# ppwwyyxx/OpenPano

Measured on AMD Instinct MI355X. Metric: SIFT keypoints+desc/sec and all-pairs matches/sec at 1/2/4/8 GPUs, higher is better.
Workload: dtype f32; 1 GPU; BASELINE config 4 restated: 38 unordered 1300x867 views per GPU (x1 GPUs = a 38-image job); seeded synthetic views (ope~; images_per_gpu=38, images_in_job=38

## Files before the change

include/openpano_hip.h:

```cpp
#ifndef OPENPANO_HIP_H
#define OPENPANO_HIP_H
#include <stddef.h>
#include <stdint.h>
#ifdef __cplusplus
extern "C" {
#endif

typedef enum {
	OP_OK = 0,
	OP_ERR_INVALID = -1,
	OP_ERR_HIP = -2,
	OP_ERR_CAPACITY = -3,
	OP_ERR_UNSUPPORTED = -4,
	OP_ERR_NO_FEATURE = -5
} op_status;

const char* op_last_error(void);
int op_abi_version(void);

typedef struct op_config {
	int SIFT_WORKING_SIZE, NUM_OCTAVE, NUM_SCALE;
	float SCALE_FACTOR, GAUSS_SIGMA;
	int GAUSS_WINDOW_FACTOR;
	float JUDGE_EXTREMA_DIFF_THRES, CONTRAST_THRES, PRE_COLOR_THRES, EDGE_RATIO;
// ... 53 lines not shown
typedef struct op_sift_dump op_sift_dump;
int op_sift_staged(op_ctx* ctx, const op_config* cfg, const op_image* img, op_sift_dump** out);
void op_sift_dump_free(op_sift_dump* d);
int op_sift_dump_working_dims(const op_sift_dump* d, int* h, int* w);
int op_sift_dump_octave_dims(const op_sift_dump* d, int oct, int* h, int* w);
int op_sift_dump_plane(op_ctx* ctx, const op_sift_dump* d, int kind, int oct, int s, float* out);
int op_sift_dump_raw_count(const op_sift_dump* d, int oct, int s);
int op_sift_dump_raw(const op_sift_dump* d, int oct, int s, int* xy);
int op_sift_dump_kp_count(const op_sift_dump* d, int which);
int op_sift_dump_kp(const op_sift_dump* d, int which, int* ints, double* real, float* fl);
int op_sift_dump_desc(const op_sift_dump* d, float* desc, double* coor);

int op_debug_math(op_ctx* ctx, int which, const float* x, const float* y, int n, float* out);
int op_debug_set_raw_capacity(op_ctx* ctx, int cap);
int op_debug_set_desc_list_cap(op_ctx* ctx, int floats);

typedef struct op_matches op_matches;
int op_match_pairs(op_ctx* ctx, const op_config* cfg, const op_features* f,
		const int* pairs, int npairs, op_matches** out);
int op_matches_count(const op_matches* m, int p);
int op_matches_copy(const op_matches* m, int p, int* idx_pairs);
int op_matches_copy_all(const op_matches* m, int* idx_pairs, int64_t* offsets);
const int* op_matches_device_list(const op_matches* m);
int64_t op_matches_total(const op_matches* m);
int op_matches_from_host(const int* const* idx_pairs, const int* counts, int npairs, op_matches** out);
int op_matches_concat(op_ctx* ctx, const op_matches* a, const op_matches* b, op_matches** out);
void op_matches_free(op_matches* m);

typedef struct op_group op_group;
int op_group_create(const int* devices, int ndev, op_group** out);
// ... 88 lines not shown
```

openpano_amd/csrc/capi.hip:

```cpp
#include "internal.hpp"
#include <cstring>

static thread_local std::string g_last_error;
void op_set_error(const std::string& msg) { g_last_error = msg; }

static hipEvent_t take_event(op_ctx* c) {
	if (!c->ev_pool.empty()) { hipEvent_t e = c->ev_pool.back(); c->ev_pool.pop_back(); return e; }
	hipEvent_t e = nullptr;
	if (hipEventCreate(&e) != hipSuccess) return nullptr;
	return e;
}
ProfScope::ProfScope(op_ctx* ctx, const char* label): c(ctx) {
	if (!c->profiling || (!c->prof_only.empty() && c->prof_only != label)) return;
	stage = c->prof_stage(label);
	a = take_event(c); b = take_event(c);
	if (a) hipEventRecord(a, c->stream);
}
ProfScope::~ProfScope() {
	if (stage < 0 || !a || !b) return;
	hipEventRecord(b, c->stream);
	c->pending.push_back({stage, a, b});
}
#include <chrono>
static double now_ms() { return std::chrono::duration<double, std::milli>(std::chrono::steady_clock::now().time_since_epoch()).count(); }
// ... 185 lines not shown
	if (n == 0) return OP_OK;
	HIPCHK(hipSetDevice(c->device));
	float *dx = nullptr, *dy = nullptr, *dout = nullptr;
	HIPCHK(hipMalloc(&dx, sizeof(float) * n));
	HIPCHK(hipMalloc(&dy, sizeof(float) * n));
	HIPCHK(hipMalloc(&dout, sizeof(float) * n));
	HIPCHK(hipMemcpyAsync(dx, x, sizeof(float) * n, hipMemcpyHostToDevice, c->stream));
	HIPCHK(hipMemcpyAsync(dy, y ? y : x, sizeof(float) * n, hipMemcpyHostToDevice, c->stream));
	HIPCHK(launch_debug_math(which, dx, dy, n, dout, c->stream));
	HIPCHK(hipMemcpyAsync(out, dout, sizeof(float) * n, hipMemcpyDeviceToHost, c->stream));
	HIPCHK(hipStreamSynchronize(c->stream));
	hipFree(dx); hipFree(dy); hipFree(dout);
	return OP_OK;
}

}
```

openpano_amd/csrc/internal.hpp:

```cpp
#pragma once
#include <hip/hip_runtime.h>
#include <stdint.h>
#include <string>
#include <vector>
#include "openpano_hip.h"

#define OP_MAX_OCT 8
#define OP_MAX_SCALE 12
#define OP_MAX_KCENTER 15

void op_set_error(const std::string& msg);
struct op_ctx;
void op_ctx_release_workspace(op_ctx* c);
#define OP_FAIL(code, msg) do { op_set_error(msg); return (code); } while (0)
#define HIPCHK(expr) do { hipError_t e_ = (expr); if (e_ != hipSuccess) { \
	op_set_error(std::string(#expr) + ": " + hipGetErrorString(e_)); return OP_ERR_HIP; } } while (0)

struct ProfStage { std::string label; double total_ms = 0; long calls = 0; };
struct op_ctx {
	int device = 0;
	int num_cu = 256;
	hipStream_t stream = nullptr;
	bool owns_stream = false;
	bool profiling = false;
// ... 64 lines not shown
#include <functional>
void host_parallel_for(int n, const std::function<void(int)>& body, int grain = 1);

hipError_t pool_alloc(void** p, size_t bytes);
void pool_free(void* p);
void pool_trim();

struct OctDesc {
	int h, w;
	int tiles_x, tiles_y, tile_begin;
	int rw_nb, rw_nseg;
	long long off;
	long long plane;
};

struct SiftPlan {
	int n;
	int sh, sw;
	int wh, ww;
	int noct, nscale;
	OctDesc oct[OP_MAX_OCT];
	int total_tiles;
	long long ws_stride;
	float* ws;
	float* work;
	const void* const* srcs;
	int src_u8;
	int* zero;
	int zero_n;
	int num_cu;
	float kern[OP_MAX_SCALE][2 * OP_MAX_KCENTER + 1];
	int kcenter[OP_MAX_SCALE];
	int halo;
	int rows_ok;
	int rw_seg;
	int rw_items;
	float kpair[3][7][2];
	float pre_color_thres, judge_thres, contrast_thres, edge_ratio, offset_thres;
	int calc_offset_depth;
	float gauss_sigma, scale_factor, ori_radius;
	int ori_smooth, desc_scale_factor, desc_int_factor;
	int desc_list_cap;
};

__host__ __device__ inline long long plane_off_grey(const OctDesc& o) { return o.off; }
// ... 6 lines not shown
	float dir, sf;
	int src;
	int pad;
};

#define OP_DESC_LIST_CAP 640
#define OP_RW_OWN 240
#define OP_RW_SEG_DEFAULT 24
#define OP_RW_SEG_MIN 16
#define OP_RW_SEG_MAX 40
#define OP_PYR_TW 64
#ifndef OP_PYR_TH
#define OP_PYR_TH 16
#endif

hipError_t launch_grey_octaves(const SiftPlan& p, bool write_work, hipStream_t st);
hipError_t launch_pyramid(const SiftPlan& p, int* raw , int* raw_count , int cap, hipStream_t st);
hipError_t launch_magort_plane(const SiftPlan& p, int img, int oct, int s, float* mag, float* ort, hipStream_t st);
hipError_t launch_refine(const SiftPlan& p, const int* raw, const int* raw_count, int cap, int expect,
		KeyPoint* refined , int* refined_count, hipStream_t st);
#define OP_OCNT_STRIDE 32
hipError_t launch_orientation(const SiftPlan& p, const KeyPoint* refined, const int* refined_count, int cap, int expect,
		float* dirs , int* ndirs , int* per_image ,
		KeyPoint* sorted , int* slot_of , hipStream_t st);
hipError_t launch_expand_oriented(const SiftPlan& p, const KeyPoint* sorted, const int* slot_of, const int* refined_count, int cap,
		const float* dirs, const int* ndirs, const int* per_image , long long* total, int* count_out ,
		KeyPoint* oriented, long long oriented_cap, hipStream_t st);
hipError_t launch_descriptor(const SiftPlan& p, const KeyPoint* oriented, const long long* total ,
		long long cap, float* desc, double* coor, double* real, hipStream_t st);
hipError_t launch_debug_math(int which, const float* x, const float* y, int n, float* out, hipStream_t st);
// ... 1 lines not shown
```

openpano_amd/csrc/pyramid.hip:

```cpp
#include "internal.hpp"
#include "devmath.hpp"

namespace {

__device__ __forceinline__ void resize_coord(int d, float inv_f, int srcn, int& s, float& r) {
	float rr = ((float)d + 0.5f) * inv_f - 0.5f;
	int ss = (int)floorf(rr);
	rr -= (float)ss;
	if (ss < 0) { ss = 0; rr = 0.f; }
	else if (ss + 1 >= srcn) { ss = srcn - 2; rr = 1.f; }
	s = ss; r = rr;
}

__device__ __forceinline__ float bilerp(float p00, float p01, float p10, float p11, float rx, float irx, float ry, float iry) {
	return rx * (p11 * ry + p10 * iry) + irx * (p01 * ry + p00 * iry);
}

#ifndef OP_GREY_WR
#define OP_GREY_WR 14
#endif
constexpr int WT = 64, WR = OP_GREY_WR;
constexpr int WP = WT + 1 + 2;

typedef float f32x4_a4 __attribute__((ext_vector_type(4), aligned(4)));
typedef float f32x2_a4 __attribute__((ext_vector_type(2), aligned(4)));
#define OP_GLOBAL __attribute__((address_space(1)))
__device__ __forceinline__ void src_run6(const float* s, long long i, const float*, float (&t)[6]) {
	const OP_GLOBAL float* g = (const OP_GLOBAL float*)s + i;
	const f32x4_a4 a = *(const OP_GLOBAL f32x4_a4*)g; const f32x2_a4 b = *(const OP_GLOBAL f32x2_a4*)(g + 4);
	t[0] = a.x; t[1] = a.y; t[2] = a.z; t[3] = a.w; t[4] = b.x; t[5] = b.y;
}
__device__ __forceinline__ void src_run6(const unsigned char* s, long long i, const float* lut, float (&t)[6]) {
#pragma unroll
	for (int k = 0; k < 6; ++k) t[k] = lut[((const OP_GLOBAL unsigned char*)s)[i + k]];
}

__device__ __forceinline__ float third(float s) { return (float)((double)s * (1.0 / 3.0)); }

constexpr int TR = 24, TC = 72;

#ifdef OP_GREY_WAVES
#define OP_GREY_ATTR __attribute__((amdgpu_waves_per_eu(OP_GREY_WAVES, OP_GREY_WAVES)))
#else
#define OP_GREY_ATTR
#endif
template <typename SrcT>
__global__ void __launch_bounds__(256) OP_GREY_ATTR k_grey_octaves(SiftPlan p, int write_work) {
	__shared__ float s_rgb[3][(WR + 1) * WP];
	__shared__ float s_lut[256];
	__shared__ int s_ri[TR], s_ci[TC];
	__shared__ float s_rw[TR], s_cw[TC];
	__shared__ long long s_ro[TR];
	const unsigned ntx = (unsigned)(p.ww + WT - 1) / WT, nty = (unsigned)(p.wh + WR - 1) / WR;
	const unsigned ntile = ntx * nty * (unsigned)p.n, per = (ntile + 7u) >> 3;
	const unsigned lin = (blockIdx.x & 7u) * per + (blockIdx.x >> 3);
	if (lin >= ntile) return;
	const int img = (int)(lin / (ntx * nty));
	const unsigned trem = lin - (unsigned)img * (ntx * nty);
	const int tx0 = (int)(trem % ntx) * WT, ty0 = (int)(trem / ntx) * WR;
	const int tid = threadIdx.x;
	const SrcT* src = (const SrcT*)p.srcs[img];
	if (blockIdx.x == 0 && p.zero)
		for (int i = tid; i < p.zero_n; i += 256) p.zero[i] = 0;
	if (sizeof(SrcT) == 1) s_lut[tid] = (float)((double)(float)tid / 255.0);
	{
		const float fx = (float)p.wh / (float)p.sh, fy = (float)p.ww / (float)p.sw;
		const float ifx = 1.f / fx, ify = 1.f / fy;
		if (tid < WR + 1) {
			int sx = -1; float rx = 0.f;
			if (ty0 + tid < p.wh) resize_coord(ty0 + tid, ifx, p.sh, sx, rx);
			s_ri[tid] = sx; s_rw[tid] = rx; s_ro[tid] = (long long)sx * p.sw * 3;
		} else if (tid >= 64 && tid < 64 + WT + 1) {
			const int c = tid - 64;
			int sy = -1; float ry = 0.f;
			if (tx0 + c < p.ww) resize_coord(tx0 + c, ify, p.sw, sy, ry);
			s_ci[c] = sy < 0 ? -1 : sy * 3; s_cw[c] = ry;
		}
		__syncthreads();
		constexpr int NE = ((WR + 1) * (WT + 1) + 255) / 256;
		float t0[NE][6], t1[NE][6];
		bool live[NE];
#pragma unroll
		for (int k = 0; k < NE; ++k) {
			const int e = tid + 256 * k < (WR + 1) * (WT + 1) ? tid + 256 * k : 0;
			const int r = e / (WT + 1), c = e % (WT + 1);
			const int sx = s_ri[r], sy3 = s_ci[c];
			live[k] = sx >= 0 && sy3 >= 0;
			const long long i0 = live[k] ? s_ro[r] + sy3 : 0, i1 = i0 + (long long)p.sw * 3;
			src_run6(src, i0, s_lut, t0[k]); src_run6(src, i1, s_lut, t1[k]);
		}
#pragma unroll
		for (int k = 0; k < NE; ++k) {
			const int e = tid + 256 * k;
			if (e >= (WR + 1) * (WT + 1)) break;
			const int r = e / (WT + 1), c = e % (WT + 1);
			float v0 = 0.f, v1 = 0.f, v2 = 0.f;
			if (live[k]) {
				const float rx = s_rw[r], ry = s_cw[c];
				const float irx = 1.0f - rx, iry = 1.0f - ry;
				v0 = bilerp(t0[k][0], t0[k][3], t1[k][0], t1[k][3], rx, irx, ry, iry);
				v1 = bilerp(t0[k][1], t0[k][4], t1[k][1], t1[k][4], rx, irx, ry, iry);
				v2 = bilerp(t0[k][2], t0[k][5], t1[k][2], t1[k][5], rx, irx, ry, iry);
				if (write_work && r < WR && c < WT) {
					float* dst = p.work + (((long long)img * p.wh + ty0 + r) * p.ww + tx0 + c) * 3;
					dst[0] = v0; dst[1] = v1; dst[2] = v2;
				}
			}
			s_rgb[0][r * WP + c] = v0; s_rgb[1][r * WP + c] = v1; s_rgb[2][r * WP + c] = v2;
		}
	}
	__syncthreads();
	float* ws = p.ws + (long long)img * p.ws_stride;
	{
		const int c = tid & (WT - 1), col = tx0 + c;
		float* g0 = ws + plane_off_grey(p.oct[0]) + (long long)ty0 * p.ww + col;
		if (col < p.ww)
			for (int r = tid >> 6; r < WR && ty0 + r < p.wh; r += 4)
				g0[(long long)r * p.ww] = third(s_rgb[0][r * WP + c] + s_rgb[1][r * WP + c] + s_rgb[2][r * WP + c]);
	}
	for (int o = 1; o < p.noct; ++o) {
		const OctDesc od = p.oct[o];
		const float fx = (float)od.h / (float)p.wh, fy = (float)od.w / (float)p.ww;
		const float ifx = 1.f / fx, ify = 1.f / fy;
		int r_lo = (int)floorf(((float)ty0 + 0.5f) * fx - 0.5f) - 1, r_hi = (int)ceilf(((float)(ty0 + WR) + 0.5f) * fx - 0.5f) + 2;
		int c_lo = (int)floorf(((float)tx0 + 0.5f) * fy - 0.5f) - 1, c_hi = (int)ceilf(((float)(tx0 + WT) + 0.5f) * fy - 0.5f) + 2;
		r_lo = r_lo < 0 ? 0 : r_lo; c_lo = c_lo < 0 ? 0 : c_lo;
		r_hi = r_hi > od.h ? od.h : r_hi; c_hi = c_hi > od.w ? od.w : c_hi;
		const int nr = r_hi - r_lo, nc = c_hi - c_lo;
		if (nr <= 0 || nc <= 0) continue;
		const bool tables = nr <= TR && nc <= TC;
		__syncthreads();
		if (tables) {
			if (tid < nr) {
				int sx; float rx;
				resize_coord(r_lo + tid, ifx, p.wh, sx, rx);
				const int lr = sx - ty0;
				s_ri[tid] = (lr >= 0 && lr < WR) ? lr : -1; s_rw[tid] = rx;
			} else if (tid >= 64 && tid - 64 < nc) {
				int sy; float ry;
				resize_coord(c_lo + tid - 64, ify, p.ww, sy, ry);
				const int lc = sy - tx0;
				s_ci[tid - 64] = (lc >= 0 && lc < WT) ? lc : -1; s_cw[tid - 64] = ry;
			}
		}
		__syncthreads();
		float* go = ws + plane_off_grey(od);
		const float inv_nc = 1.0f / (float)nc;
		for (int e = tid; e < nr * nc; e += 256) {
			int q = (int)(((float)e + 0.5f) * inv_nc), rem = e - q * nc;
			if (rem < 0) { --q; rem += nc; } else if (rem >= nc) { ++q; rem -= nc; }
			const int dr = r_lo + q, dc = c_lo + rem;
			int lr, lc; float rx, ry;
			if (tables) { lr = s_ri[q]; lc = s_ci[rem]; rx = s_rw[q]; ry = s_cw[rem]; }
			else {
				int sx, sy;
				resize_coord(dr, ifx, p.wh, sx, rx);
				resize_coord(dc, ify, p.ww, sy, ry);
				lr = sx - ty0; lc = sy - tx0;
				if (lr >= WR) lr = -1;
				if (lc >= WT) lc = -1;
			}
			if (lr < 0 || lc < 0) continue;
			const float irx = 1.0f - rx, iry = 1.0f - ry;
			const int b = lr * WP + lc;
			const float r = bilerp(s_rgb[0][b], s_rgb[0][b + 1], s_rgb[0][b + WP], s_rgb[0][b + WP + 1], rx, irx, ry, iry);
			const float g = bilerp(s_rgb[1][b], s_rgb[1][b + 1], s_rgb[1][b + WP], s_rgb[1][b + WP + 1], rx, irx, ry, iry);
			const float bl = bilerp(s_rgb[2][b], s_rgb[2][b + 1], s_rgb[2][b + WP], s_rgb[2][b + WP + 1], rx, irx, ry, iry);
			go[(long long)dr * od.w + dc] = third(r + g + bl);
		}
	}
}

constexpr int TW = OP_PYR_TW, TH = OP_PYR_TH;
constexpr int GR = TH + 2, GC = TW + 2;
constexpr int PG = TH == 16 ? 75 : GC + 1;
constexpr int PV = GR + (GR % 2 == 0 ? 1 : 2);
constexpr int NPX = TW * TH / 256;
constexpr int NHALO = 2 * GC + 2 * TH;
static_assert(TW == 64 && TH % 4 == 0 && NHALO <= 256, "tile shape");
constexpr int RV = TH == 32 ? 12 : (TH == 24 ? 9 : 6);
constexpr int RH = TH == 32 ? 10 : (TH == 24 ? 8 : 6);
static_assert(((GR + RV - 1) / RV) * (GC + 12) <= 256 && ((GC + RH - 1) / RH) * GR <= 256, "blocking must fit 256 threads at halo 6");

// ... 575 lines not shown
		case 2: r = opdev::sinf_glibc(x[i]); break;
		case 3: r = opdev::hypotf_glibc(x[i], y[i]); break;
		default: r = opdev::fast_atan_plus_pi(y[i], x[i]); break;
	}
	out[i] = r;
}

}

size_t pyramid_lds_bytes(int halo) {
	const int NR = GR + 2 * halo, NC = GC + 2 * halo;
	return sizeof(float) * ((size_t)NR * NC + (size_t)vt_rows(halo) * PV + 4 * (size_t)GR * PG);
}

hipError_t launch_grey_octaves(const SiftPlan& p, bool write_work, hipStream_t st) {
	const unsigned ntile = (unsigned)((p.ww + WT - 1) / WT) * (unsigned)((p.wh + WR - 1) / WR) * (unsigned)p.n;
	dim3 grid(((ntile + 7u) >> 3) << 3);
	if (p.src_u8) hipLaunchKernelGGL(k_grey_octaves<unsigned char>, grid, dim3(256), 0, st, p, write_work ? 1 : 0);
	else hipLaunchKernelGGL(k_grey_octaves<float>, grid, dim3(256), 0, st, p, write_work ? 1 : 0);
	return hipGetLastError();
}

hipError_t launch_magort_plane(const SiftPlan& p, int img, int oct, int s, float* mag, float* ort, hipStream_t st) {
	const long long n = p.oct[oct].plane;
	hipLaunchKernelGGL(k_magort_plane, dim3((unsigned)((n + 255) / 256)), dim3(256), 0, st, p, img, oct, s, mag, ort);
	return hipGetLastError();
}

hipError_t launch_pyramid(const SiftPlan& p, int* raw, int* raw_count, int cap, hipStream_t st) {
	size_t lds = pyramid_lds_bytes(p.halo);
	{
// ... 20 lines not shown
```

openpano_amd/csrc/sift_host.hip:

```cpp
#include "internal.hpp"
#include <algorithm>
#include <array>
#include <cmath>
#include <cstring>
#include <map>
#include <memory>
#include <mutex>
#include <thread>

size_t pyramid_lds_bytes(int halo);

namespace {

struct DevBuf {
	void* p = nullptr; size_t cap = 0;
	hipError_t ensure(size_t bytes) {
		if (bytes <= cap) return hipSuccess;
		if (p) { hipError_t e = hipFree(p); if (e != hipSuccess) return e; p = nullptr; cap = 0; }
		size_t want = bytes + bytes / 8;
		hipError_t e = hipMalloc(&p, want);
		if (e != hipSuccess) return e;
		cap = want;
		return hipSuccess;
	}
	void release() { if (p) hipFree(p); p = nullptr; cap = 0; }
};

}

struct Workspace {
	DevBuf ws, work, srcs, staging, raw, counts, refinedA, refinedB, slot_of, dirs, ndirs, oriented;
	void* pinned = nullptr; size_t pinned_cap = 0;
	std::vector<const void*> srcs_last; void* srcs_dev = nullptr;
	long long last_total = 0;
	int last_raw_max = 0, last_refined_max = 0;
	int raw_cap = 16384;
	int desc_list_cap = OP_DESC_LIST_CAP;
	void release() {
		ws.release(); work.release(); srcs.release(); staging.release(); raw.release(); counts.release();
		refinedA.release(); refinedB.release(); slot_of.release(); dirs.release(); ndirs.release(); oriented.release();
		if (pinned) hipHostFree(pinned); pinned = nullptr; pinned_cap = 0;
		srcs_last.clear(); srcs_dev = nullptr;
	}
};

static std::map<op_ctx*, Workspace*> g_ws;
static std::mutex g_ws_mu;

static Workspace* ctx_workspace(op_ctx* c) {
	std::lock_guard<std::mutex> lk(g_ws_mu);
	auto it = g_ws.find(c);
	if (it != g_ws.end()) return it->second;
	Workspace* w = new Workspace;
	g_ws[c] = w;
	return w;
// ... 67 lines not shown
		kernel[0] = 1;
		float exp_coeff = (float)(-1.0 / (sigma * sigma * 2)), wsum = 1;
		for (int i = 1; i <= center; i++)
			wsum += (kernel[i] = std::exp((float)(i * i) * exp_coeff)) * 2;
		float fac = (float)(1.0 / wsum);
		kernel[0] = fac;
		for (int i = 1; i <= center; i++)
			kernel[-i] = (kernel[i] *= fac);
		p.kcenter[s] = center;
		p.halo = std::max(p.halo, center);
		sigma *= cfg.SCALE_FACTOR;
	}
	return 0;
}

int build_plan(const op_config& cfg, int n, int sh, int sw, SiftPlan& p, int num_cu = 256) {
	memset(&p, 0, sizeof(p));
	if (cfg.NUM_OCTAVE < 1 || cfg.NUM_OCTAVE > OP_MAX_OCT || cfg.NUM_SCALE < 4 || cfg.NUM_SCALE > OP_MAX_SCALE)
		OP_FAIL(OP_ERR_UNSUPPORTED, "NUM_OCTAVE must be in [1,8] and NUM_SCALE in [4,12]");
	if (sh < 2 || sw < 2) OP_FAIL(OP_ERR_INVALID, "image must be at least 2x2 (lib/imgproc.cc:321)");
	p.n = n; p.sh = sh; p.sw = sw;
	float ratio = cfg.SIFT_WORKING_SIZE * 2.0f / (sw + sh);
	p.wh = (int)(sh * ratio); p.ww = (int)(sw * ratio);
	if (p.wh < 2 || p.ww < 2) OP_FAIL(OP_ERR_INVALID, "working image degenerate");
	p.noct = cfg.NUM_OCTAVE; p.nscale = cfg.NUM_SCALE;
	long long off = 0; int tile_begin = 0;
	for (int i = 0; i < p.noct; ++i) {
		OctDesc& o = p.oct[i];
		if (i == 0) { o.h = p.wh; o.w = p.ww; }
		else {
			float factor = (float)std::pow((double)cfg.SCALE_FACTOR, (double)-i);
			o.w = (int)std::ceil(p.ww * factor); o.h = (int)std::ceil(p.wh * factor);
			if (!(o.w > 5 && o.h > 5)) OP_FAIL(OP_ERR_INVALID, "octave smaller than 6 px (feature/dog.cc:108 assertion)");
		}
		o.plane = (long long)o.h * o.w;
		o.off = off; off += o.plane * planes_per_octave(p.nscale);
		o.tiles_x = (o.w + OP_PYR_TW - 1) / OP_PYR_TW; o.tiles_y = (o.h + OP_PYR_TH - 1) / OP_PYR_TH;
		o.tile_begin = tile_begin; tile_begin += o.tiles_x * o.tiles_y;
	}
	p.total_tiles = tile_begin;
	p.ws_stride = (off + 63) & ~63LL;
	if (build_gauss_bank(cfg, p) != 0) OP_FAIL(OP_ERR_UNSUPPORTED, "Gaussian kernel wider than 31 taps");
	{
		static const int shipped[6] = {3, 3, 3, 6, 6, 6};
		p.rows_ok = p.nscale == 7;
		for (int s = 1; s < 7 && p.rows_ok; ++s) if (p.kcenter[s] != shipped[s - 1]) p.rows_ok = 0;
		if (p.rows_ok) {
			auto items_at = [&](int seg) {
				long long it = 0;
				for (int i = 0; i < p.noct; ++i) it += (long long)((p.oct[i].w + OP_RW_OWN - 1) / OP_RW_OWN) * ((p.oct[i].h + seg - 1) / seg);
				return it;
			};
			int seg = OP_RW_SEG_DEFAULT;
#ifdef OP_RW_SEG
			seg = OP_RW_SEG;
// ... 61 lines not shown
	HIPCHK(W.raw.ensure(sizeof(int) * 4 * (size_t)cap * n));
	const size_t cnt_hdr = ((3 * (size_t)n + 2) + 31) & ~(size_t)31;
	HIPCHK(W.counts.ensure(sizeof(int) * (cnt_hdr + (size_t)n * OP_OCNT_STRIDE)));
	HIPCHK(W.refinedA.ensure(sizeof(KeyPoint) * (size_t)cap * n));
	HIPCHK(W.refinedB.ensure(sizeof(KeyPoint) * (size_t)cap * n));
	HIPCHK(W.dirs.ensure(sizeof(float) * 36 * (size_t)cap * n));
	HIPCHK(W.ndirs.ensure(sizeof(int) * (size_t)cap * n));
	HIPCHK(W.slot_of.ensure(sizeof(int) * (size_t)cap * n));
	const size_t pin_need = sizeof(long long) * (size_t)(8 * n + 16);
	if (W.pinned_cap < pin_need) {
		if (W.pinned) hipHostFree(W.pinned);
		HIPCHK(hipHostMalloc(&W.pinned, pin_need));
		W.pinned_cap = pin_need;
	}
	plan.ws = (float*)W.ws.p; plan.work = (float*)W.work.p;

	plan.src_u8 = imgs[0]->dtype == OP_U8 ? 1 : 0;
	const size_t img_bytes = (plan.src_u8 ? 1 : sizeof(float)) * (size_t)sh * sw * 3;
	const size_t img_stride = (img_bytes + 255) & ~(size_t)255;
	size_t host_bytes = 0;
	for (auto* im : imgs) if (!im->on_device) host_bytes += img_stride;
	if (host_bytes) HIPCHK(W.staging.ensure(host_bytes));
	{
		const void** hs = (const void**)W.pinned;
		bool packed = host_bytes == img_stride * (size_t)n && n > 1;
		ptrdiff_t hstride = 0;
		if (packed) hstride = (const char*)imgs[1]->data - (const char*)imgs[0]->data;
		packed = packed && hstride >= (ptrdiff_t)img_bytes;
		for (int i = 2; i < n && packed; ++i) packed = (const char*)imgs[i]->data - (const char*)imgs[i - 1]->data == hstride;
		if (packed) {
// ... 79 lines not shown
		if (raw_count[0]) HIPCHK(hipMemcpy(keep->raw.data(), W.raw.p, sizeof(int) * 4 * raw_count[0], hipMemcpyDeviceToHost));
		keep->refined.resize(refined_count[0]);
		if (refined_count[0]) HIPCHK(hipMemcpy(keep->refined.data(), W.refinedB.p, sizeof(KeyPoint) * refined_count[0], hipMemcpyDeviceToHost));
		keep->oriented.resize(total);
		if (total) HIPCHK(hipMemcpy(keep->oriented.data(), W.oriented.p, sizeof(KeyPoint) * total, hipMemcpyDeviceToHost));
		keep->desc.resize((size_t)total * 128);
		if (total) HIPCHK(hipMemcpy(keep->desc.data(), res.desc, sizeof(float) * 128 * total, hipMemcpyDeviceToHost));
		std::vector<std::array<int, 4>> q(raw_count[0]);
		for (int i = 0; i < raw_count[0]; ++i) q[i] = {keep->raw[4 * i + 2], keep->raw[4 * i + 3], keep->raw[4 * i + 1], keep->raw[4 * i]};
		std::sort(q.begin(), q.end());
		for (int i = 0; i < raw_count[0]; ++i) { keep->raw[4 * i] = q[i][3]; keep->raw[4 * i + 1] = q[i][2]; keep->raw[4 * i + 2] = q[i][0]; keep->raw[4 * i + 3] = q[i][1]; }
	}
	return OP_OK;
}

}

extern "C" {

int op_sift_batch(op_ctx* ctx, const op_config* cfg, const op_image* imgs, int n, op_features** out) {
	if (!ctx || !cfg || !imgs || n <= 0 || !out) OP_FAIL(OP_ERR_INVALID, "op_sift_batch: bad argument");
	HIPCHK(hipSetDevice(ctx->device));
	for (int i = 0; i < n; ++i)
		if (!imgs[i].data || imgs[i].h < 2 || imgs[i].w < 2 || (imgs[i].dtype != OP_F32 && imgs[i].dtype != OP_U8))
			OP_FAIL(OP_ERR_INVALID, "op_sift_batch: bad image " + std::to_string(i));
	std::vector<std::pair<std::pair<int, int>, std::vector<int>>> groups;
	for (int i = 0; i < n; ++i) {
		std::pair<int, int> key(imgs[i].h * 2 + imgs[i].dtype, imgs[i].w);
		bool found = false;
		for (auto& g : groups) if (g.first == key) { g.second.push_back(i); found = true; break; }
// ... 402 lines not shown
```

openpano_amd/hip.py:

```python
from __future__ import annotations

import ctypes as C
import os

import numpy as np

_HERE = os.path.dirname(os.path.abspath(__file__))
LIB_PATH = os.environ.get("OPENPANO_HIP_LIB") or os.path.join(_HERE, "libopenpano_hip.so")


class OpenPanoHipError(RuntimeError):
    pass


class OpConfig(C.Structure):
    _fields_ = [
        ("SIFT_WORKING_SIZE", C.c_int), ("NUM_OCTAVE", C.c_int), ("NUM_SCALE", C.c_int),
        ("SCALE_FACTOR", C.c_float), ("GAUSS_SIGMA", C.c_float), ("GAUSS_WINDOW_FACTOR", C.c_int),
        ("JUDGE_EXTREMA_DIFF_THRES", C.c_float), ("CONTRAST_THRES", C.c_float),
        ("PRE_COLOR_THRES", C.c_float), ("EDGE_RATIO", C.c_float),
        ("CALC_OFFSET_DEPTH", C.c_int), ("OFFSET_THRES", C.c_float),
        ("ORI_RADIUS", C.c_float), ("ORI_HIST_SMOOTH_COUNT", C.c_int),
        ("DESC_HIST_SCALE_FACTOR", C.c_int), ("DESC_INT_FACTOR", C.c_int),
        ("MATCH_REJECT_NEXT_RATIO", C.c_float), ("RANSAC_ITERATIONS", C.c_int),
# ... 91 lines not shown
        L.op_features_adopt_device.argtypes = [C.c_void_p, C.c_void_p, C.c_void_p, C.POINTER(C.c_int), C.c_int, C.POINTER(C.c_void_p)]
    L.op_features_free.argtypes = [C.c_void_p]
    L.op_sift_staged.argtypes = [C.c_void_p, C.POINTER(OpConfig), C.POINTER(OpImage), C.POINTER(C.c_void_p)]
    L.op_sift_dump_free.argtypes = [C.c_void_p]
    L.op_sift_dump_working_dims.argtypes = [C.c_void_p, C.POINTER(C.c_int), C.POINTER(C.c_int)]
    L.op_sift_dump_octave_dims.argtypes = [C.c_void_p, C.c_int, C.POINTER(C.c_int), C.POINTER(C.c_int)]
    L.op_sift_dump_plane.argtypes = [C.c_void_p, C.c_void_p, C.c_int, C.c_int, C.c_int, C.c_void_p]
    L.op_sift_dump_raw_count.argtypes = [C.c_void_p, C.c_int, C.c_int]
    L.op_sift_dump_raw.argtypes = [C.c_void_p, C.c_int, C.c_int, C.c_void_p]
    L.op_sift_dump_kp_count.argtypes = [C.c_void_p, C.c_int]
    L.op_sift_dump_kp.argtypes = [C.c_void_p, C.c_int, C.c_void_p, C.c_void_p, C.c_void_p]
    L.op_sift_dump_desc.argtypes = [C.c_void_p, C.c_void_p, C.c_void_p]
    L.op_debug_math.argtypes = [C.c_void_p, C.c_int, C.c_void_p, C.c_void_p, C.c_int, C.c_void_p]
    L.op_debug_set_raw_capacity.argtypes = [C.c_void_p, C.c_int]
    L.op_debug_set_desc_list_cap.argtypes = [C.c_void_p, C.c_int]
    if hasattr(L, "op_match_pairs"):
        L.op_match_pairs.argtypes = [C.c_void_p, C.POINTER(OpConfig), C.c_void_p, C.c_void_p, C.c_int, C.POINTER(C.c_void_p)]
        L.op_matches_count.argtypes = [C.c_void_p, C.c_int]
        L.op_matches_copy.argtypes = [C.c_void_p, C.c_int, C.c_void_p]
        if hasattr(L, "op_matches_copy_all"):
            L.op_matches_copy_all.argtypes = [C.c_void_p, C.c_void_p, C.c_void_p]
        if hasattr(L, "op_matches_device_list"):
            L.op_matches_device_list.restype = C.c_void_p
        if hasattr(L, "op_matches_device_list"):
            L.op_matches_device_list.argtypes = [C.c_void_p]
        L.op_matches_total.restype = C.c_int64
        L.op_matches_total.argtypes = [C.c_void_p]
        L.op_matches_free.argtypes = [C.c_void_p]
    L.op_group_create.argtypes = [C.POINTER(C.c_int), C.c_int, C.POINTER(C.c_void_p)]
    L.op_group_destroy.argtypes = [C.c_void_p]
# ... 817 lines not shown
```

Before: 51.04 million keypoints+descriptors/s.

## Precompute octave resize tables on host for grey-octave kernel

Moves per-tile octave downsample coordinate and weight computation in k_grey_octaves into host-built tables. The tables are cached per geometry and uploaded once, then fetched from constant address space into LDS. Tile index division now uses magic-number multiplies, and source and store addressing uses 32-bit byte offsets. This removes per-block resize_coord math and several barriers, at the cost of a new device buffer, a sync on geometry change, and a limit on source images of 4 GiB or more.

```diff
diff --git a/include/openpano_hip.h b/include/openpano_hip.h
--- a/include/openpano_hip.h
+++ b/include/openpano_hip.h
@@ -91,6 +91,7 @@
 int op_debug_math(op_ctx* ctx, int which, const float* x, const float* y, int n, float* out);
 int op_debug_set_raw_capacity(op_ctx* ctx, int cap);
 int op_debug_set_desc_list_cap(op_ctx* ctx, int floats);
+int op_debug_grey_tables(const op_config* cfg, int sh, int sw, int* hdr, int32_t* words, int64_t cap_words);
 
 typedef struct op_matches op_matches;
 int op_match_pairs(op_ctx* ctx, const op_config* cfg, const op_features* f,
diff --git a/openpano_amd/csrc/capi.hip b/openpano_amd/csrc/capi.hip
--- a/openpano_amd/csrc/capi.hip
+++ b/openpano_amd/csrc/capi.hip
@@ -223,4 +223,16 @@
 	return OP_OK;
 }
 
-}
+int op_debug_grey_tables(const op_config* cfg, int sh, int sw, int* hdr, int32_t* words, int64_t cap_words) {
+	if (!cfg || !hdr || cap_words < 0) OP_FAIL(OP_ERR_INVALID, "op_debug_grey_tables: bad argument");
+	std::vector<int32_t> t;
+	const int rc = grey_tables_debug(*cfg, sh, sw, hdr, t);
+	if (rc != OP_OK) return rc;
+	if (words) {
+		if ((int64_t)t.size() > cap_words) OP_FAIL(OP_ERR_CAPACITY, "op_debug_grey_tables: " + std::to_string(t.size()) + " words, room for " + std::to_string(cap_words));
+		memcpy(words, t.data(), sizeof(int32_t) * t.size());
+	}
+	return OP_OK;
+}
+
+}
diff --git a/openpano_amd/csrc/internal.hpp b/openpano_amd/csrc/internal.hpp
--- a/openpano_amd/csrc/internal.hpp
+++ b/openpano_amd/csrc/internal.hpp
@@ -102,6 +102,21 @@
 	long long plane;
 };
 
+#define OP_GREY_WT 64
+#ifndef OP_GREY_WR
+#define OP_GREY_WR 14
+#endif
+#define OP_GREY_TR 24
+#define OP_GREY_TC 72
+struct GreyTabs {
+	const int* base;
+	int words;
+	int ntx, nty;
+	unsigned tpi, m_tpi, m_ntx;
+	float ifx, ify;
+	int orow[OP_MAX_OCT], ocol[OP_MAX_OCT], rrun[OP_MAX_OCT], crun[OP_MAX_OCT];
+};
+
 struct SiftPlan {
 	int n;
 	int sh, sw;
@@ -117,6 +132,7 @@
 	int* zero;
 	int zero_n;
 	int num_cu;
+	GreyTabs gt;
 	float kern[OP_MAX_SCALE][2 * OP_MAX_KCENTER + 1];
 	int kcenter[OP_MAX_SCALE];
 	int halo;
@@ -153,6 +169,8 @@
 #define OP_PYR_TH 16
 #endif
 
+int grey_tables_debug(const op_config& cfg, int sh, int sw, int* hdr, std::vector<int32_t>& words);
+
 hipError_t launch_grey_octaves(const SiftPlan& p, bool write_work, hipStream_t st);
 hipError_t launch_pyramid(const SiftPlan& p, int* raw , int* raw_count , int cap, hipStream_t st);
 hipError_t launch_magort_plane(const SiftPlan& p, int img, int oct, int s, float* mag, float* ort, hipStream_t st);
diff --git a/openpano_amd/csrc/pyramid.hip b/openpano_amd/csrc/pyramid.hip
--- a/openpano_amd/csrc/pyramid.hip
+++ b/openpano_amd/csrc/pyramid.hip
@@ -2,6 +2,38 @@
 #include "devmath.hpp"
 
 namespace {
+
+__device__ __forceinline__ float bilerp(float p00, float p01, float p10, float p11, float rx, float irx, float ry, float iry) {
+	return rx * (p11 * ry + p10 * iry) + irx * (p01 * ry + p00 * iry);
+}
+
+constexpr int WT = OP_GREY_WT, WR = OP_GREY_WR;
+constexpr int WP = WT + 1 + 2;
+static_assert(WT == 64, "k_grey_octaves: thread = column in the octave-0 pass");
+
+#define OP_GLOBAL __attribute__((address_space(1)))
+#define OP_CONST __attribute__((address_space(4)))
+typedef int i32x2 __attribute__((ext_vector_type(2)));
+typedef int i32x4 __attribute__((ext_vector_type(4)));
+template <typename T>
+__device__ __forceinline__ T gload(const OP_CONST void* base, unsigned byte_off) { return *(const OP_CONST T*)((const OP_CONST char*)base + byte_off); }
+__device__ __forceinline__ void gstore(OP_GLOBAL void* base, unsigned byte_off, float v) { *(OP_GLOBAL float*)((OP_GLOBAL char*)base + byte_off) = v; }
+typedef float f32x4_a4 __attribute__((ext_vector_type(4), aligned(4)));
+typedef float f32x2_a4 __attribute__((ext_vector_type(2), aligned(4)));
+__device__ __forceinline__ void src_run6(const OP_GLOBAL float* s, unsigned i, const float*, float (&t)[6]) {
+	const OP_GLOBAL char* g = (const OP_GLOBAL char*)s + i;
+	const f32x4_a4 a = *(const OP_GLOBAL f32x4_a4*)g; const f32x2_a4 b = *(const OP_GLOBAL f32x2_a4*)(g + 16);
+	t[0] = a.x; t[1] = a.y; t[2] = a.z; t[3] = a.w; t[4] = b.x; t[5] = b.y;
+}
+__device__ __forceinline__ void src_run6(const OP_GLOBAL unsigned char* s, unsigned i, const float* lut, float (&t)[6]) {
+	const OP_GLOBAL unsigned char* g = s + i;
+#pragma unroll
+	for (int k = 0; k < 6; ++k) t[k] = lut[g[k]];
+}
+
+__device__ __forceinline__ float third(float s) { return (float)((double)s * (1.0 / 3.0)); }
+
+constexpr int TR = OP_GREY_TR, TC = OP_GREY_TC;
 
 __device__ __forceinline__ void resize_coord(int d, float inv_f, int srcn, int& s, float& r) {
 	float rr = ((float)d + 0.5f) * inv_f - 0.5f;
@@ -12,32 +44,12 @@
 	s = ss; r = rr;
 }
 
-__device__ __forceinline__ float bilerp(float p00, float p01, float p10, float p11, float rx, float irx, float ry, float iry) {
-	return rx * (p11 * ry + p10 * iry) + irx * (p01 * ry + p00 * iry);
-}
-
-#ifndef OP_GREY_WR
-#define OP_GREY_WR 14
-#endif
-constexpr int WT = 64, WR = OP_GREY_WR;
-constexpr int WP = WT + 1 + 2;
-
-typedef float f32x4_a4 __attribute__((ext_vector_type(4), aligned(4)));
-typedef float f32x2_a4 __attribute__((ext_vector_type(2), aligned(4)));
-#define OP_GLOBAL __attribute__((address_space(1)))
-__device__ __forceinline__ void src_run6(const float* s, long long i, const float*, float (&t)[6]) {
-	const OP_GLOBAL float* g = (const OP_GLOBAL float*)s + i;
-	const f32x4_a4 a = *(const OP_GLOBAL f32x4_a4*)g; const f32x2_a4 b = *(const OP_GLOBAL f32x2_a4*)(g + 4);
-	t[0] = a.x; t[1] = a.y; t[2] = a.z; t[3] = a.w; t[4] = b.x; t[5] = b.y;
-}
-__device__ __forceinline__ void src_run6(const unsigned char* s, long long i, const float* lut, float (&t)[6]) {
-#pragma unroll
-	for (int k = 0; k < 6; ++k) t[k] = lut[((const OP_GLOBAL unsigned char*)s)[i + k]];
-}
-
-__device__ __forceinline__ float third(float s) { return (float)((double)s * (1.0 / 3.0)); }
-
-constexpr int TR = 24, TC = 72;
+__device__ __forceinline__ unsigned udiv_magic(unsigned x, unsigned d, unsigned m, unsigned& rem) {
+	unsigned q = __umulhi(x, m), r = x - q * d;
+	if (r >= d) { ++q; r -= d; }
+	rem = r;
+	return q;
+}
 
 #ifdef OP_GREY_WAVES
 #define OP_GREY_ATTR __attribute__((amdgpu_waves_per_eu(OP_GREY_WAVES, OP_GREY_WAVES)))
@@ -48,46 +60,57 @@
 __global__ void __launch_bounds__(256) OP_GREY_ATTR k_grey_octaves(SiftPlan p, int write_work) {
 	__shared__ float s_rgb[3][(WR + 1) * WP];
 	__shared__ float s_lut[256];
-	__shared__ int s_ri[TR], s_ci[TC];
-	__shared__ float s_rw[TR], s_cw[TC];
-	__shared__ long long s_ro[TR];
-	const unsigned ntx = (unsigned)(p.ww + WT - 1) / WT, nty = (unsigned)(p.wh + WR - 1) / WR;
-	const unsigned ntile = ntx * nty * (unsigned)p.n, per = (ntile + 7u) >> 3;
+	__shared__ i32x2 s_ot[OP_MAX_OCT - 1][TR + TC];
+	const unsigned ntile = p.gt.tpi * (unsigned)p.n, per = (ntile + 7u) >> 3;
 	const unsigned lin = (blockIdx.x & 7u) * per + (blockIdx.x >> 3);
 	if (lin >= ntile) return;
-	const int img = (int)(lin / (ntx * nty));
-	const unsigned trem = lin - (unsigned)img * (ntx * nty);
-	const int tx0 = (int)(trem % ntx) * WT, ty0 = (int)(trem / ntx) * WR;
+	unsigned trem, txi;
+	const int img = (int)udiv_magic(lin, p.gt.tpi, p.gt.m_tpi, trem);
+	const unsigned tyi = udiv_magic(trem, (unsigned)p.gt.ntx, p.gt.m_ntx, txi);
+	const int tx0 = (int)txi * WT, ty0 = (int)tyi * WR;
 	const int tid = threadIdx.x;
-	const SrcT* src = (const SrcT*)p.srcs[img];
+	const OP_GLOBAL SrcT* src = (const OP_GLOBAL SrcT*)p.srcs[img];
+	const OP_CONST int* gt = (const OP_CONST int*)p.gt.base;
 	if (blockIdx.x == 0 && p.zero)
 		for (int i = tid; i < p.zero_n; i += 256) p.zero[i] = 0;
 	if (sizeof(SrcT) == 1) s_lut[tid] = (float)((double)(float)tid / 255.0);
 	{
-		const float fx = (float)p.wh / (float)p.sh, fy = (float)p.ww / (float)p.sw;
-		const float ifx = 1.f / fx, ify = 1.f / fy;
-		if (tid < WR + 1) {
-			int sx = -1; float rx = 0.f;
-			if (ty0 + tid < p.wh) resize_coord(ty0 + tid, ifx, p.sh, sx, rx);
-			s_ri[tid] = sx; s_rw[tid] = rx; s_ro[tid] = (long long)sx * p.sw * 3;
-		} else if (tid >= 64 && tid < 64 + WT + 1) {
-			const int c = tid - 64;
-			int sy = -1; float ry = 0.f;
-			if (tx0 + c < p.ww) resize_coord(tx0 + c, ify, p.sw, sy, ry);
-			s_ci[c] = sy < 0 ? -1 : sy * 3; s_cw[c] = ry;
-		}
-		__syncthreads();
 		constexpr int NE = ((WR + 1) * (WT + 1) + 255) / 256;
-		float t0[NE][6], t1[NE][6];
+		const OP_GLOBAL SrcT* src1 = src + (unsigned)p.sw * 3u;
+		float t0[NE][6], t1[NE][6], wr[NE], wc[NE];
 		bool live[NE];
+		if (sizeof(SrcT) == 1) __syncthreads();
 #pragma unroll
 		for (int k = 0; k < NE; ++k) {
 			const int e = tid + 256 * k < (WR + 1) * (WT + 1) ? tid + 256 * k : 0;
 			const int r = e / (WT + 1), c = e % (WT + 1);
-			const int sx = s_ri[r], sy3 = s_ci[c];
-			live[k] = sx >= 0 && sy3 >= 0;
-			const long long i0 = live[k] ? s_ro[r] + sy3 : 0, i1 = i0 + (long long)p.sw * 3;
-			src_run6(src, i0, s_lut, t0[k]); src_run6(src, i1, s_lut, t1[k]);
+			int sx = -1, sy = -1;
+			wr[k] = 0.f; wc[k] = 0.f;
+			if (ty0 + r < p.wh) resize_coord(ty0 + r, p.gt.ifx, p.sh, sx, wr[k]);
+			if (tx0 + c < p.ww) resize_coord(tx0 + c, p.gt.ify, p.sw, sy, wc[k]);
+			live[k] = sx >= 0 && sy >= 0;
+			const unsigned i0 = live[k] ? (unsigned)((sx * p.sw + sy) * 3) * (unsigned)sizeof(SrcT) : 0u;
+			src_run6(src, i0, s_lut, t0[k]); src_run6(src1, i0, s_lut, t1[k]);
+		}
+		{
+			const bool cols = tid >= 64;
+			const int li = cols ? tid - 64 : tid, slot = cols ? TR + li : li;
+			auto fetch = [&](int o, bool& has) -> i32x2 {
+				const i32x4 rr = *(const OP_CONST i32x4*)(gt + p.gt.rrun[o] + 4 * (int)tyi), cr = *(const OP_CONST i32x4*)(gt + p.gt.crun[o] + 4 * (int)txi);
+				const int at_r = __builtin_amdgcn_readfirstlane(p.gt.orow[o] + 2 * rr.x), at_c = __builtin_amdgcn_readfirstlane(p.gt.ocol[o] + 2 * cr.x);
+				has = li < (cols ? cr.y : rr.y);
+				i32x2 v = {0, 0};
+				if (has) v = gload<i32x2>(gt, (unsigned)((cols ? at_c : at_r) + 2 * li) * 4u);
+				return v;
+			};
+			bool has = false, has_next = false;
+			i32x2 ent = {0, 0}, next = {0, 0};
+			if (p.noct > 1) ent = fetch(1, has);
+			for (int o = 1; o < p.noct; ++o) {
+				if (o + 1 < p.noct) next = fetch(o + 1, has_next);
+				if (has) s_ot[o - 1][slot] = ent;
+				ent = next; has = has_next;
+			}
 		}
 #pragma unroll
 		for (int k = 0; k < NE; ++k) {
@@ -96,7 +119,7 @@
 			const int r = e / (WT + 1), c = e % (WT + 1);
 			float v0 = 0.f, v1 = 0.f, v2 = 0.f;
 			if (live[k]) {
-				const float rx = s_rw[r], ry = s_cw[c];
+				const float rx = wr[k], ry = wc[k];
 				const float irx = 1.0f - rx, iry = 1.0f - ry;
 				v0 = bilerp(t0[k][0], t0[k][3], t1[k][0], t1[k][3], rx, irx, ry, iry);
 				v1 = bilerp(t0[k][1], t0[k][4], t1[k][1], t1[k][4], rx, irx, ry, iry);
@@ -110,63 +133,30 @@
 		}
 	}
 	__syncthreads();
-	float* ws = p.ws + (long long)img * p.ws_stride;
+	OP_GLOBAL float* ws = (OP_GLOBAL float*)p.ws + (long long)img * p.ws_stride;
 	{
-		const int c = tid & (WT - 1), col = tx0 + c;
-		float* g0 = ws + plane_off_grey(p.oct[0]) + (long long)ty0 * p.ww + col;
-		if (col < p.ww)
-			for (int r = tid >> 6; r < WR && ty0 + r < p.wh; r += 4)
-				g0[(long long)r * p.ww] = third(s_rgb[0][r * WP + c] + s_rgb[1][r * WP + c] + s_rgb[2][r * WP + c]);
-	}
+		const int c = tid & (WT - 1);
+		OP_GLOBAL float* g0 = ws + plane_off_grey(p.oct[0]) + (long long)ty0 * p.ww + tx0;
+		const int rows = p.wh - ty0 < WR ? p.wh - ty0 : WR;
+		if (tx0 + c < p.ww)
+			for (int r = tid >> 6; r < rows; r += 4)
+				gstore(g0, (unsigned)(r * p.ww + c) * 4u, third(s_rgb[0][r * WP + c] + s_rgb[1][r * WP + c] + s_rgb[2][r * WP + c]));
+	}
+	const int lds0 = ty0 * WP + tx0;
 	for (int o = 1; o < p.noct; ++o) {
-		const OctDesc od = p.oct[o];
-		const float fx = (float)od.h / (float)p.wh, fy = (float)od.w / (float)p.ww;
-		const float ifx = 1.f / fx, ify = 1.f / fy;
-		int r_lo = (int)floorf(((float)ty0 + 0.5f) * fx - 0.5f) - 1, r_hi = (int)ceilf(((float)(ty0 + WR) + 0.5f) * fx - 0.5f) + 2;
-		int c_lo = (int)floorf(((float)tx0 + 0.5f) * fy - 0.5f) - 1, c_hi = (int)ceilf(((float)(tx0 + WT) + 0.5f) * fy - 0.5f) + 2;
-		r_lo = r_lo < 0 ? 0 : r_lo; c_lo = c_lo < 0 ? 0 : c_lo;
-		r_hi = r_hi > od.h ? od.h : r_hi; c_hi = c_hi > od.w ? od.w : c_hi;
-		const int nr = r_hi - r_lo, nc = c_hi - c_lo;
-		if (nr <= 0 || nc <= 0) continue;
-		const bool tables = nr <= TR && nc <= TC;
-		__syncthreads();
-		if (tables) {
-			if (tid < nr) {
-				int sx; float rx;
-				resize_coord(r_lo + tid, ifx, p.wh, sx, rx);
-				const int lr = sx - ty0;
-				s_ri[tid] = (lr >= 0 && lr < WR) ? lr : -1; s_rw[tid] = rx;
-			} else if (tid >= 64 && tid - 64 < nc) {
-				int sy; float ry;
-				resize_coord(c_lo + tid - 64, ify, p.ww, sy, ry);
-				const int lc = sy - tx0;
-				s_ci[tid - 64] = (lc >= 0 && lc < WT) ? lc : -1; s_cw[tid - 64] = ry;
-			}
-		}
-		__syncthreads();
-		float* go = ws + plane_off_grey(od);
-		const float inv_nc = 1.0f / (float)nc;
-		for (int e = tid; e < nr * nc; e += 256) {
-			int q = (int)(((float)e + 0.5f) * inv_nc), rem = e - q * nc;
-			if (rem < 0) { --q; rem += nc; } else if (rem >= nc) { ++q; rem -= nc; }
-			const int dr = r_lo + q, dc = c_lo + rem;
-			int lr, lc; float rx, ry;
-			if (tables) { lr = s_ri[q]; lc = s_ci[rem]; rx = s_rw[q]; ry = s_cw[rem]; }
-			else {
-				int sx, sy;
-				resize_coord(dr, ifx, p.wh, sx, rx);
-				resize_coord(dc, ify, p.ww, sy, ry);
-				lr = sx - ty0; lc = sy - tx0;
-				if (lr >= WR) lr = -1;
-				if (lc >= WT) lc = -1;
-			}
-			if (lr < 0 || lc < 0) continue;
+		const i32x4 rr = *(const OP_CONST i32x4*)(gt + p.gt.rrun[o] + 4 * (int)tyi), cr = *(const OP_CONST i32x4*)(gt + p.gt.crun[o] + 4 * (int)txi);
+		const int nc = cr.y, ne = rr.y * nc, ow = p.oct[o].w;
+		OP_GLOBAL float* go = ws + plane_off_grey(p.oct[o]) + (long long)rr.x * ow + cr.x;
+		for (int e = tid; e < ne; e += 256) {
+			const int q = (int)__umulhi(2u * (unsigned)e, (unsigned)cr.z), rem = e - q * nc;
+			const i32x2 re = s_ot[o - 1][q], ce = s_ot[o - 1][TR + rem];
+			const float rx = __int_as_float(re.y), ry = __int_as_float(ce.y);
 			const float irx = 1.0f - rx, iry = 1.0f - ry;
-			const int b = lr * WP + lc;
+			const int b = re.x * WP + ce.x - lds0;
 			const float r = bilerp(s_rgb[0][b], s_rgb[0][b + 1], s_rgb[0][b + WP], s_rgb[0][b + WP + 1], rx, irx, ry, iry);
 			const float g = bilerp(s_rgb[1][b], s_rgb[1][b + 1], s_rgb[1][b + WP], s_rgb[1][b + WP + 1], rx, irx, ry, iry);
 			const float bl = bilerp(s_rgb[2][b], s_rgb[2][b + 1], s_rgb[2][b + WP], s_rgb[2][b + WP + 1], rx, irx, ry, iry);
-			go[(long long)dr * od.w + dc] = third(r + g + bl);
+			gstore(go, (unsigned)(q * ow + rem) * 4u, third(r + g + bl));
 		}
 	}
 }
@@ -772,7 +762,8 @@
 }
 
 hipError_t launch_grey_octaves(const SiftPlan& p, bool write_work, hipStream_t st) {
-	const unsigned ntile = (unsigned)((p.ww + WT - 1) / WT) * (unsigned)((p.wh + WR - 1) / WR) * (unsigned)p.n;
+	if (!p.gt.base) return hipErrorInvalidValue;
+	const unsigned ntile = p.gt.tpi * (unsigned)p.n;
 	dim3 grid(((ntile + 7u) >> 3) << 3);
 	if (p.src_u8) hipLaunchKernelGGL(k_grey_octaves<unsigned char>, grid, dim3(256), 0, st, p, write_work ? 1 : 0);
 	else hipLaunchKernelGGL(k_grey_octaves<float>, grid, dim3(256), 0, st, p, write_work ? 1 : 0);
diff --git a/openpano_amd/csrc/sift_host.hip b/openpano_amd/csrc/sift_host.hip
--- a/openpano_amd/csrc/sift_host.hip
+++ b/openpano_amd/csrc/sift_host.hip
@@ -29,9 +29,11 @@
 }
 
 struct Workspace {
-	DevBuf ws, work, srcs, staging, raw, counts, refinedA, refinedB, slot_of, dirs, ndirs, oriented;
+	DevBuf ws, work, srcs, staging, raw, counts, refinedA, refinedB, slot_of, dirs, ndirs, oriented, greytab;
 	void* pinned = nullptr; size_t pinned_cap = 0;
 	std::vector<const void*> srcs_last; void* srcs_dev = nullptr;
+	std::array<int, 8 + 2 * OP_MAX_OCT> grey_key{}; bool grey_valid = false;
+	std::vector<int32_t> grey_host;
 	long long last_total = 0;
 	int last_raw_max = 0, last_refined_max = 0;
 	int raw_cap = 16384;
@@ -39,6 +41,7 @@
 	void release() {
 		ws.release(); work.release(); srcs.release(); staging.release(); raw.release(); counts.release();
 		refinedA.release(); refinedB.release(); slot_of.release(); dirs.release(); ndirs.release(); oriented.release();
+		greytab.release(); grey_valid = false;
 		if (pinned) hipHostFree(pinned); pinned = nullptr; pinned_cap = 0;
 		srcs_last.clear(); srcs_dev = nullptr;
 	}
@@ -136,6 +139,67 @@
 	return 0;
 }
 
+inline void resize_coord(int d, float inv_f, int srcn, int& s, float& r) {
+	float rr = ((float)d + 0.5f) * inv_f - 0.5f;
+	int ss = (int)floorf(rr);
+	rr -= (float)ss;
+	if (ss < 0) { ss = 0; rr = 0.f; }
+	else if (ss + 1 >= srcn) { ss = srcn - 2; rr = 1.f; }
+	s = ss; r = rr;
+}
+
+unsigned div_magic(unsigned d) { return d <= 1 ? 0xFFFFFFFFu : (unsigned)((1ull << 32) / d); }
+
+void grey_tables_layout(SiftPlan& p) {
+	GreyTabs& g = p.gt;
+	g.base = nullptr;
+	g.ntx = (p.ww + OP_GREY_WT - 1) / OP_GREY_WT; g.nty = (p.wh + OP_GREY_WR - 1) / OP_GREY_WR;
+	g.tpi = (unsigned)g.ntx * (unsigned)g.nty; g.m_tpi = div_magic(g.tpi); g.m_ntx = div_magic((unsigned)g.ntx);
+	{ const float fx = (float)p.wh / (float)p.sh, fy = (float)p.ww / (float)p.sw; g.ifx = 1.f / fx; g.ify = 1.f / fy; }
+	int w = 0;
+	auto take = [&](int words) { const int at = w; w += (words + 3) & ~3; return at; };
+	for (int o = 1; o < p.noct; ++o) {
+		g.orow[o] = take(2 * p.oct[o].h); g.ocol[o] = take(2 * p.oct[o].w);
+		g.rrun[o] = take(4 * g.nty); g.crun[o] = take(4 * g.ntx);
+	}
+	g.words = w > 0 ? w : 4;
+}
+
+int grey_tables_fill(const SiftPlan& p, std::vector<int32_t>& t) {
+	const GreyTabs& g = p.gt;
+	t.assign((size_t)g.words, 0);
+	auto bits = [](float f) { int32_t i; memcpy(&i, &f, sizeof(i)); return i; };
+	for (int o = 1; o < p.noct; ++o) {
+		const OctDesc& od = p.oct[o];
+		const float fx = (float)od.h / (float)p.wh, fy = (float)od.w / (float)p.ww;
+		const float ifx = 1.f / fx, ify = 1.f / fy;
+		int max_run[2] = {0, 0};
+		for (int axis = 0; axis < 2; ++axis) {
+			const int nd = axis ? od.w : od.h, srcn = axis ? p.ww : p.wh, tile = axis ? OP_GREY_WT : OP_GREY_WR, ntile = axis ? g.ntx : g.nty;
+			int32_t* tab = &t[(size_t)(axis ? g.ocol[o] : g.orow[o])];
+			int32_t* run = &t[(size_t)(axis ? g.crun[o] : g.rrun[o])];
+			for (int d = 0; d < nd; ++d) {
+				int sx; float rx;
+				resize_coord(d, axis ? ify : ifx, srcn, sx, rx);
+				if (d && sx < tab[2 * (d - 1)]) OP_FAIL(OP_ERR_UNSUPPORTED, "octave coordinates are not monotonic");
+				tab[2 * d] = sx; tab[2 * d + 1] = bits(rx);
+			}
+			int d = 0;
+			for (int ti = 0; ti < ntile; ++ti) {
+				const int first = d;
+				while (d < nd && tab[2 * d] < (ti + 1) * tile) ++d;
+				const int count = d - first;
+				run[4 * ti] = first; run[4 * ti + 1] = count;
+				run[4 * ti + 2] = count ? (int32_t)(uint32_t)(((1ull << 31) + (unsigned)count - 1) / (unsigned)count) : 0;
+				max_run[axis] = std::max(max_run[axis], count);
+			}
+		}
+		if (max_run[0] > OP_GREY_TR || max_run[1] > OP_GREY_TC || max_run[0] * max_run[1] >= 32768)
+			OP_FAIL(OP_ERR_UNSUPPORTED, "octave " + std::to_string(o) + " is larger than the working image (SCALE_FACTOR < 1)");
+	}
+	return OP_OK;
+}
+
 int build_plan(const op_config& cfg, int n, int sh, int sw, SiftPlan& p, int num_cu = 256) {
 	memset(&p, 0, sizeof(p));
 	if (cfg.NUM_OCTAVE < 1 || cfg.NUM_OCTAVE > OP_MAX_OCT || cfg.NUM_SCALE < 4 || cfg.NUM_SCALE > OP_MAX_SCALE)
@@ -145,6 +209,7 @@
 	float ratio = cfg.SIFT_WORKING_SIZE * 2.0f / (sw + sh);
 	p.wh = (int)(sh * ratio); p.ww = (int)(sw * ratio);
 	if (p.wh < 2 || p.ww < 2) OP_FAIL(OP_ERR_INVALID, "working image degenerate");
+	if (12ull * (unsigned)sw * (unsigned)sh > 0xFFFFFF00ull) OP_FAIL(OP_ERR_UNSUPPORTED, "source image of 4 GiB or more (k_grey_octaves addresses it with 32-bit byte offsets)");
 	p.noct = cfg.NUM_OCTAVE; p.nscale = cfg.NUM_SCALE;
 	long long off = 0; int tile_begin = 0;
 	for (int i = 0; i < p.noct; ++i) {
@@ -161,6 +226,7 @@
 		o.tile_begin = tile_begin; tile_begin += o.tiles_x * o.tiles_y;
 	}
 	p.total_tiles = tile_begin;
+	grey_tables_layout(p);
 	p.ws_stride = (off + 63) & ~63LL;
 	if (build_gauss_bank(cfg, p) != 0) OP_FAIL(OP_ERR_UNSUPPORTED, "Gaussian kernel wider than 31 taps");
 	{
@@ -252,6 +318,21 @@
 		W.pinned_cap = pin_need;
 	}
 	plan.ws = (float*)W.ws.p; plan.work = (float*)W.work.p;
+	{
+		std::array<int, 8 + 2 * OP_MAX_OCT> key{};
+		key[0] = sh; key[1] = sw; key[2] = plan.wh; key[3] = plan.ww; key[4] = plan.noct; key[5] = OP_GREY_WT; key[6] = OP_GREY_WR; key[7] = plan.gt.words;
+		for (int o = 0; o < plan.noct; ++o) { key[8 + 2 * o] = plan.oct[o].h; key[9 + 2 * o] = plan.oct[o].w; }
+		if (!W.grey_valid || key != W.grey_key) {
+			W.grey_valid = false;
+			HIPCHK(hipStreamSynchronize(st));
+			rc = grey_tables_fill(plan, W.grey_host);
+			if (rc != OP_OK) return rc;
+			HIPCHK(W.greytab.ensure(sizeof(int32_t) * W.grey_host.size()));
+			HIPCHK(hipMemcpyAsync(W.greytab.p, W.grey_host.data(), sizeof(int32_t) * W.grey_host.size(), hipMemcpyHostToDevice, st));
+			W.grey_key = key; W.grey_valid = true;
+		}
+		plan.gt.base = (const int*)W.greytab.p;
+	}
 
 	plan.src_u8 = imgs[0]->dtype == OP_U8 ? 1 : 0;
 	const size_t img_bytes = (plan.src_u8 ? 1 : sizeof(float)) * (size_t)sh * sw * 3;
@@ -361,6 +442,23 @@
 	return OP_OK;
 }
 
+}
+
+int grey_tables_debug(const op_config& cfg, int sh, int sw, int* hdr, std::vector<int32_t>& words) {
+	SiftPlan p;
+	int rc = build_plan(cfg, 1, sh, sw, p);
+	if (rc != OP_OK) return rc;
+	rc = grey_tables_fill(p, words);
+	if (rc != OP_OK) return rc;
+	const GreyTabs& g = p.gt;
+	memset(hdr, 0, sizeof(int) * 64);
+	hdr[0] = g.words; hdr[1] = p.wh; hdr[2] = p.ww; hdr[3] = p.noct; hdr[4] = OP_GREY_WT; hdr[5] = OP_GREY_WR;
+	hdr[6] = g.ntx; hdr[7] = g.nty; memcpy(&hdr[8], &g.ifx, sizeof(float)); memcpy(&hdr[9], &g.ify, sizeof(float));
+	for (int o = 0; o < p.noct; ++o) {
+		int* h = hdr + 16 + 6 * o;
+		h[0] = p.oct[o].h; h[1] = p.oct[o].w; h[2] = g.orow[o]; h[3] = g.ocol[o]; h[4] = g.rrun[o]; h[5] = g.crun[o];
+	}
+	return OP_OK;
 }
 
 extern "C" {
diff --git a/openpano_amd/hip.py b/openpano_amd/hip.py
--- a/openpano_amd/hip.py
+++ b/openpano_amd/hip.py
@@ -129,6 +129,8 @@
     L.op_debug_math.argtypes = [C.c_void_p, C.c_int, C.c_void_p, C.c_void_p, C.c_int, C.c_void_p]
     L.op_debug_set_raw_capacity.argtypes = [C.c_void_p, C.c_int]
     L.op_debug_set_desc_list_cap.argtypes = [C.c_void_p, C.c_int]
+    if hasattr(L, "op_debug_grey_tables"):
+        L.op_debug_grey_tables.argtypes = [C.POINTER(OpConfig), C.c_int, C.c_int, C.POINTER(C.c_int), C.c_void_p, C.c_int64]
     if hasattr(L, "op_match_pairs"):
         L.op_match_pairs.argtypes = [C.c_void_p, C.POINTER(OpConfig), C.c_void_p, C.c_void_p, C.c_int, C.POINTER(C.c_void_p)]
         L.op_matches_count.argtypes = [C.c_void_p, C.c_int]
```

Result: faster. 51.71 million keypoints+descriptors/s, median of 4 (+1.3%).
